# MasterBin-IIAU/Unicorn

Hardware: NVIDIA H100
Metric: frames/sec (higher is better)
Workload: dtype bf16

## Files before the change

unicorn_b200/csrc/mlp_fused.cu:

```cuda
#include <algorithm>
#include "uc_ptx.cuh"
#include "uc_common.h"
#include "../../include/unicorn_b200.h"
#include "uc_epilogue.cuh"

namespace uc {

constexpr int kMlpRows = 128;
constexpr int kMlpHC = 64;
constexpr int kMlpConsumers = 2;
constexpr int kMlpThreads = (1 + kMlpConsumers) * 128;

template <int C>
struct MlpCfg {
  static constexpr int KB = (C + 63) / 64;
  static constexpr int A_BYTES = KB * kMlpRows * 128;
  static constexpr int W1_BYTES = KB * kMlpHC * 128;
  static constexpr int NH = C > 256 ? 2 : 1;
  static constexpr int N2 = C / NH;
  static constexpr int W2_BYTES = N2 * 128;
  static constexpr int NCHUNK = 4 * C / kMlpHC;
  static constexpr int STEPS = NH * NCHUNK;
  static constexpr int AS = C <= 192 ? 2 : 1;
  static constexpr int WS = C <= 256 ? 2 : 1;
  static constexpr int SMEM = AS * A_BYTES + WS * (W1_BYTES + W2_BYTES) + 1024 + 512;
  static constexpr int CPT = C / 16;
};

struct alignas(64) MlpParams {
  CUtensorMap tmA, tmW1, tmW2;
  const float* c1;
  const float* b2;
  const float* gamma;
  uint16_t* x;
  int M, m_tiles;
  float ln_eps;
};

enum { A_FULL = 0, A_EMPTY = 2, W1_FULL = 4, W1_EMPTY = 6, W2_FULL = 8, W2_EMPTY = 10, MLP_NBARS = 12 };

template <int C>
__global__ void __launch_bounds__(kMlpThreads, 1) convnext_mlp_kernel(const __grid_constant__ MlpParams p) {
  using Cfg = MlpCfg<C>;
  extern __shared__ uint8_t smem_raw[];
  uint8_t* smem = reinterpret_cast<uint8_t*>((reinterpret_cast<uintptr_t>(smem_raw) + 1023) & ~uintptr_t(1023));
  uint8_t* sA = smem;
  uint8_t* sW1 = sA + Cfg::AS * Cfg::A_BYTES;
  uint8_t* sW2 = sW1 + Cfg::WS * Cfg::W1_BYTES;
  uint64_t* bar = reinterpret_cast<uint64_t*>(sW2 + Cfg::WS * Cfg::W2_BYTES);
  const int wg = threadIdx.x >> 7, warp = threadIdx.x >> 5, lane = threadIdx.x & 31;

  if (threadIdx.x == 0) {
    prefetch_tmap(&p.tmA);
    prefetch_tmap(&p.tmW1);
    prefetch_tmap(&p.tmW2);
    for (int i = 0; i < 2; ++i) {
      mbar_init(&bar[A_FULL + i], 1);
      mbar_init(&bar[A_EMPTY + i], kMlpConsumers);
      mbar_init(&bar[W1_FULL + i], 1);
      mbar_init(&bar[W1_EMPTY + i], kMlpConsumers);
      mbar_init(&bar[W2_FULL + i], 1);
      mbar_init(&bar[W2_EMPTY + i], kMlpConsumers);
    }
    fence_barrier_init();
  }
  __syncthreads();
  pdl_wait();
  pdl_launch_dependents();

  const int n_local = (p.m_tiles - static_cast<int>(blockIdx.x) + static_cast<int>(gridDim.x) - 1) / static_cast<int>(gridDim.x);
  auto tile_of = [&](int i) { return static_cast<int>(blockIdx.x) + i * static_cast<int>(gridDim.x); };

  if (wg == 0) {
    regs_dealloc<40>();
    if (warp != 0) return;
    auto load_a = [&](int i) {
      const int ab = i % Cfg::AS;
      mbar_wait(&bar[A_EMPTY + ab], ((i / Cfg::AS) & 1) ^ 1);
      if (elect_one()) {
        mbar_arrive_expect_tx(&bar[A_FULL + ab], Cfg::A_BYTES);
#pragma unroll
        for (int kb = 0; kb < Cfg::KB; ++kb)
          tma_load_2d(sA + ab * Cfg::A_BYTES + kb * (kMlpRows * 128), &p.tmA, &bar[A_FULL + ab], kb * 64, tile_of(i) * kMlpRows);
      }
      __syncwarp();
    };
    auto load_w = [&](int g) {
      const int s = g % Cfg::WS, ph = (g / Cfg::WS) & 1, j = g % Cfg::NCHUNK, nh = (g / Cfg::NCHUNK) % Cfg::NH;
      mbar_wait(&bar[W1_EMPTY + s], ph ^ 1);
      if (elect_one()) {
        mbar_arrive_expect_tx(&bar[W1_FULL + s], Cfg::W1_BYTES);
#pragma unroll
        for (int kb = 0; kb < Cfg::KB; ++kb)
          tma_load_2d(sW1 + s * Cfg::W1_BYTES + kb * (kMlpHC * 128), &p.tmW1, &bar[W1_FULL + s], kb * 64, j * kMlpHC);
      }
      __syncwarp();
      mbar_wait(&bar[W2_EMPTY + s], ph ^ 1);
      if (elect_one()) {
        mbar_arrive_expect_tx(&bar[W2_FULL + s], Cfg::W2_BYTES);
        tma_load_2d(sW2 + s * Cfg::W2_BYTES, &p.tmW2, &bar[W2_FULL + s], j * kMlpHC, nh * Cfg::N2);
      }
      __syncwarp();
    };
    const int total = n_local * Cfg::STEPS;
    if (n_local > 0) load_a(0);
    for (int g = 0; g < total; ++g) {
      load_w(g);
      const int i = g / Cfg::STEPS, r = g % Cfg::STEPS;
      if (r == (Cfg::AS == 2 ? 0 : Cfg::STEPS - 1) && i + 1 < n_local) load_a(i + 1);
    }
    return;
  }
  regs_alloc<232>();
  const int c = wg - 1, ct = threadIdx.x & 127;
  const int g8 = lane >> 2, t = lane & 3;
  const int rl = (warp & 3) * 16 + g8;
  const int lr = c * 64 + (ct >> 1), lp = ct & 1;
  auto layer_norm_tile = [&](int ab) {
    uint8_t* a = sA + ab * Cfg::A_BYTES + lr * 128;
    auto chunk_ptr = [&](int cc) {
      const int gc = lp * Cfg::CPT + cc;
      return reinterpret_cast<uint4*>(a + (gc >> 3) * (kMlpRows * 128) + (((gc & 7) ^ (lr & 7)) << 4));
    };
    float s1 = 0.f;
#pragma unroll 4
    for (int cc = 0; cc < Cfg::CPT; ++cc) {
      const uint4 v = *chunk_ptr(cc);
      s1 += (bf16lo(v.x) + bf16hi(v.x)) + (bf16lo(v.y) + bf16hi(v.y)) + (bf16lo(v.z) + bf16hi(v.z)) + (bf16lo(v.w) + bf16hi(v.w));
    }
    s1 += __shfl_xor_sync(0xffffffffu, s1, 1);
    const float mean = s1 * (1.f / C);
    float s2 = 0.f;
#pragma unroll 4
    for (int cc = 0; cc < Cfg::CPT; ++cc) {
      const uint4 v = *chunk_ptr(cc);
      const uint32_t w[4] = {v.x, v.y, v.z, v.w};
#pragma unroll
      for (int e = 0; e < 4; ++e) {
        const float d0 = bf16lo(w[e]) - mean, d1 = bf16hi(w[e]) - mean;
        s2 = fmaf(d0, d0, s2);
        s2 = fmaf(d1, d1, s2);
      }
    }
    s2 += __shfl_xor_sync(0xffffffffu, s2, 1);
    const float rstd = rsqrtf(s2 * (1.f / C) + p.ln_eps);
#pragma unroll 4
    for (int cc = 0; cc < Cfg::CPT; ++cc) {
      uint4* ptr = chunk_ptr(cc);
      const uint4 v = *ptr;
      const uint32_t w[4] = {v.x, v.y, v.z, v.w};
      uint32_t o[4];
#pragma unroll
      for (int e = 0; e < 4; ++e) o[e] = pack2_fast((bf16lo(w[e]) - mean) * rstd, (bf16hi(w[e]) - mean) * rstd, false);
      *ptr = make_uint4(o[0], o[1], o[2], o[3]);
    }
    fence_proxy_async();
    named_sync(1 + c, 128);
  };
  const uint64_t a_desc0 = wgmma_desc_sw128(smem_u32(sA + c * 64 * 128)), w1_desc0 = wgmma_desc_sw128(smem_u32(sW1));
  const uint64_t w2_desc0 = wgmma_desc_sw128(smem_u32(sW2));
  float acc2[Cfg::N2 / 2];
  int g = 0;
  for (int i = 0; i < n_local; ++i) {
    const int ab = i % Cfg::AS;
    mbar_wait(&bar[A_FULL + ab], (i / Cfg::AS) & 1);
    layer_norm_tile(ab);
#pragma unroll 1
   for (int nh = 0; nh < Cfg::NH; ++nh) {
    for (int j = 0; j < Cfg::NCHUNK; ++j, ++g) {
      const int ws = g % Cfg::WS, wph = (g / Cfg::WS) & 1;
      float acc1[kMlpHC / 2];
      mbar_wait(&bar[W1_FULL + ws], wph);
      wgmma_fence();
#pragma unroll
      for (int kb = 0; kb < Cfg::KB; ++kb) {
        const uint64_t ad = a_desc0 + static_cast<uint64_t>((ab * Cfg::A_BYTES + kb * (kMlpRows * 128)) >> 4);
        const uint64_t bd = w1_desc0 + static_cast<uint64_t>((ws * Cfg::W1_BYTES + kb * (kMlpHC * 128)) >> 4);
#pragma unroll
        for (int k = 0; k < 4; ++k) wgmma_ss<kMlpHC, false>(acc1, ad + 2 * k, bd + 2 * k, (kb | k) != 0 ? 1u : 0u);
      }
      wgmma_commit();
      wgmma_wait<0>();
      wgmma_fence_regs(acc1);
      if (ct == 0) {
        mbar_arrive(&bar[W1_EMPTY + ws]);
        if (nh == Cfg::NH - 1 && j == Cfg::NCHUNK - 1) mbar_arrive(&bar[A_EMPTY + ab]);
      }
      uint32_t hf[4][4];
#pragma unroll
      for (int kk = 0; kk < 4; ++kk) {
#pragma unroll
        for (int half = 0; half < 2; ++half) {
          const int i8 = 2 * kk + half;
          const float2 bb = __ldg(reinterpret_cast<const float2*>(p.c1 + j * kMlpHC + 8 * i8 + 2 * t));
          const f32x2 h0 = gelu2(add2(pk2(acc1[4 * i8], acc1[4 * i8 + 1]), pk2(bb.x, bb.y)));
          const f32x2 h1 = gelu2(add2(pk2(acc1[4 * i8 + 2], acc1[4 * i8 + 3]), pk2(bb.x, bb.y)));
          hf[kk][2 * half] = pack2_fast(lo2(h0), hi2(h0), false);
          hf[kk][2 * half + 1] = pack2_fast(lo2(h1), hi2(h1), false);
        }
      }
      mbar_wait(&bar[W2_FULL + ws], wph);
      wgmma_fence();
      const uint64_t bd2 = w2_desc0 + static_cast<uint64_t>((ws * Cfg::W2_BYTES) >> 4);
#pragma unroll
      for (int kk = 0; kk < 4; ++kk) wgmma_rs_bf16<Cfg::N2>(acc2, hf[kk], bd2 + 2 * kk, (j | kk) != 0 ? 1u : 0u);
      wgmma_commit();
      wgmma_wait<0>();
      wgmma_fence_regs(acc2);
      if (ct == 0) mbar_arrive(&bar[W2_EMPTY + ws]);
    }
    const long grow0 = static_cast<long>(tile_of(i)) * kMlpRows + c * 64 + rl;
#pragma unroll
    for (int i8 = 0; i8 < Cfg::N2 / 8; ++i8) {
      const int col = nh * Cfg::N2 + 8 * i8 + 2 * t;
      const float2 b = __ldg(reinterpret_cast<const float2*>(p.b2 + col)), gm = __ldg(reinterpret_cast<const float2*>(p.gamma + col));
#pragma unroll
      for (int h = 0; h < 2; ++h) {
        const long grow = grow0 + 8 * h;
        if (grow < p.M) {
          uint32_t* xp = reinterpret_cast<uint32_t*>(p.x + grow * C + col);
          const uint32_t rw = *xp;
          f32x2 v = add2(pk2(acc2[4 * i8 + 2 * h], acc2[4 * i8 + 2 * h + 1]), pk2(b.x, b.y));
          v = mul2(v, pk2(gm.x, gm.y));
          v = add2(v, pk2(bf16lo(rw), bf16hi(rw)));
          *xp = pack2_fast(lo2(v), hi2(v), false);
        }
      }
    }
   }
  }
}

template <int C>
static int launch_mlp(MlpParams& p, cudaStream_t stream) {
  using Cfg = MlpCfg<C>;
  static PerDeviceFlag attr_dev;
  bool& attr = attr_dev.get();
  auto kern = convnext_mlp_kernel<C>;
  if (!attr) {
    cudaError_t e = cudaFuncSetAttribute(kern, cudaFuncAttributeMaxDynamicSharedMemorySize, Cfg::SMEM);
    if (e != cudaSuccess) return set_error(static_cast<int>(e), "uc_convnext_mlp: cudaFuncSetAttribute: %s", cudaGetErrorString(e));
    attr = true;
  }
  const int grid = std::min(p.m_tiles, num_sms());
  cudaError_t e = launch_pdl(kern, dim3(grid), dim3(kMlpThreads), Cfg::SMEM, stream, p);
  if (e != cudaSuccess) return set_error(static_cast<int>(e), "uc_convnext_mlp<%d> launch: %s", C, cudaGetErrorString(e));
  return check_launch("uc_convnext_mlp");
}

}

using namespace uc;

extern "C" int uc_convnext_mlp_supported(int C) { return C == 96 || C == 192 || C == 256 || C == 384; }

extern "C" int uc_convnext_mlp(const void* t_bf16, const void* w1f_bf16, const float* c1, const void* w2_bf16, const float* b2,
                               const float* gamma, void* x_bf16, int M, int C, float ln_eps, void* stream_v) {
  cudaStream_t stream = static_cast<cudaStream_t>(stream_v);
  if (!t_bf16 || !w1f_bf16 || !c1 || !w2_bf16 || !b2 || !gamma || !x_bf16) return set_error(UC_EINVAL, "uc_convnext_mlp: null pointer");
  if (!uc_convnext_mlp_supported(C)) return set_error(UC_EINVAL, "uc_convnext_mlp: C = %d not supported (96, 192, 256, 384)", C);
  if (M < 1) return set_error(UC_EINVAL, "uc_convnext_mlp: empty map");
  if ((reinterpret_cast<uintptr_t>(t_bf16) | reinterpret_cast<uintptr_t>(w1f_bf16) | reinterpret_cast<uintptr_t>(w2_bf16)) & 15 ||
      (reinterpret_cast<uintptr_t>(x_bf16) | reinterpret_cast<uintptr_t>(c1) | reinterpret_cast<uintptr_t>(b2) | reinterpret_cast<uintptr_t>(gamma)) & 31)
    return set_error(UC_EINVAL, "uc_convnext_mlp: t / weights 16-byte, x / biases 32-byte aligned");
  if (t_bf16 == x_bf16) return set_error(UC_EINVAL, "uc_convnext_mlp: t and x must be different maps");
  int rc = ensure_driver();
  if (rc) return rc;
  MlpParams p;
  memset(&p, 0, sizeof(p));
  const uint64_t es = 2;
  {
    uint64_t dims[2] = {static_cast<uint64_t>(C), static_cast<uint64_t>(M)};
    uint64_t strides[1] = {static_cast<uint64_t>(C) * es};
    uint32_t box[2] = {64, kMlpRows};
    rc = encode_tmap(&p.tmA, CU_TENSOR_MAP_DATA_TYPE_BFLOAT16, 2, t_bf16, dims, strides, box);
    if (rc) return rc;
  }
  {
    uint64_t dims[2] = {static_cast<uint64_t>(C), static_cast<uint64_t>(4 * C)};
    uint64_t strides[1] = {static_cast<uint64_t>(C) * es};
    uint32_t box[2] = {64, kMlpHC};
    rc = encode_tmap(&p.tmW1, CU_TENSOR_MAP_DATA_TYPE_BFLOAT16, 2, w1f_bf16, dims, strides, box);
    if (rc) return rc;
  }
  {
    uint64_t dims[2] = {static_cast<uint64_t>(4 * C), static_cast<uint64_t>(C)};
    uint64_t strides[1] = {static_cast<uint64_t>(4 * C) * es};
    uint32_t box[2] = {kMlpHC, static_cast<uint32_t>(C > 256 ? C / 2 : C)};
    rc = encode_tmap(&p.tmW2, CU_TENSOR_MAP_DATA_TYPE_BFLOAT16, 2, w2_bf16, dims, strides, box);
    if (rc) return rc;
  }
  p.c1 = c1; p.b2 = b2; p.gamma = gamma;
  p.x = static_cast<uint16_t*>(x_bf16);
  p.M = M;
  p.m_tiles = (M + kMlpRows - 1) / kMlpRows;
  p.ln_eps = ln_eps;
  return C == 96 ? launch_mlp<96>(p, stream) : C == 192 ? launch_mlp<192>(p, stream) : C == 256 ? launch_mlp<256>(p, stream) : launch_mlp<384>(p, stream);
}
```

unicorn_b200/csrc/uc_ptx.cuh:

```cuda
#pragma once
#include <cuda_runtime.h>
#include <cuda_bf16.h>
#include <cuda_fp16.h>
#include <cuda.h>
#include <stdint.h>
#include <stdio.h>
#include "uc_wgmma.cuh"

namespace uc {

__device__ __forceinline__ uint32_t smem_u32(const void* p) {
  return static_cast<uint32_t>(__cvta_generic_to_shared(p));
}

__device__ __forceinline__ bool elect_one() {
  uint32_t pred;
  asm volatile(
      "{\n\t.reg .pred p;\n\t"
      "elect.sync _|p, 0xffffffff;\n\t"
      "selp.u32 %0, 1, 0, p;\n\t}"
      : "=r"(pred));
  return pred != 0;
}

__device__ __forceinline__ void mbar_init(uint64_t* bar, uint32_t count) {
  asm volatile("mbarrier.init.shared::cta.b64 [%0], %1;" ::"r"(smem_u32(bar)), "r"(count) : "memory");
}
__device__ __forceinline__ void fence_barrier_init() {
  asm volatile("fence.mbarrier_init.release.cluster;" ::: "memory");
}
__device__ __forceinline__ void fence_proxy_async() {
  asm volatile("fence.proxy.async.shared::cta;" ::: "memory");
}
__device__ __forceinline__ void mbar_arrive_expect_tx(uint64_t* bar, uint32_t bytes) {
  asm volatile("mbarrier.arrive.expect_tx.shared::cta.b64 _, [%0], %1;" ::"r"(smem_u32(bar)), "r"(bytes)
               : "memory");
}
__device__ __forceinline__ void mbar_arrive(uint64_t* bar) {
  asm volatile("mbarrier.arrive.shared::cta.b64 _, [%0];" ::"r"(smem_u32(bar)) : "memory");
}
__device__ __forceinline__ bool mbar_try_wait(uint64_t* bar, uint32_t parity) {
  uint32_t ok;
  asm volatile(
      "{\n\t.reg .pred p;\n\t"
      "mbarrier.try_wait.parity.shared::cta.b64 p, [%1], %2;\n\t"
      "selp.u32 %0, 1, 0, p;\n\t}"
      : "=r"(ok)
      : "r"(smem_u32(bar)), "r"(parity)
      : "memory");
  return ok != 0;
}
__device__ __forceinline__ void mbar_wait(uint64_t* bar, uint32_t parity) {
  if (mbar_try_wait(bar, parity)) return;
  long long t0 = clock64();
  uint32_t spins = 0;
  while (!mbar_try_wait(bar, parity)) {
    if ((++spins & 0x3FF) == 0 && (clock64() - t0) > 4000000000LL) __trap();
  }
}

__device__ __forceinline__ void prefetch_tmap(const CUtensorMap* m) {
  asm volatile("prefetch.tensormap [%0];" ::"l"(reinterpret_cast<uint64_t>(m)) : "memory");
}
__device__ __forceinline__ void tma_load_2d(void* smem, const CUtensorMap* m, uint64_t* bar, int c0, int c1) {
  asm volatile(
      "cp.async.bulk.tensor.2d.shared::cluster.global.mbarrier::complete_tx::bytes [%0], [%1, {%3, %4}], [%2];" ::"r"(
          smem_u32(smem)),
      "l"(reinterpret_cast<uint64_t>(m)), "r"(smem_u32(bar)), "r"(c0), "r"(c1)
      : "memory");
}
__device__ __forceinline__ void tma_load_3d(void* smem, const CUtensorMap* m, uint64_t* bar, int c0, int c1, int c2) {
  asm volatile(
      "cp.async.bulk.tensor.3d.shared::cluster.global.mbarrier::complete_tx::bytes [%0], [%1, {%3, %4, %5}], [%2];" ::
          "r"(smem_u32(smem)),
      "l"(reinterpret_cast<uint64_t>(m)), "r"(smem_u32(bar)), "r"(c0), "r"(c1), "r"(c2)
      : "memory");
}
__device__ __forceinline__ void tma_load_4d(void* smem, const CUtensorMap* m, uint64_t* bar, int c0, int c1, int c2,
                                            int c3) {
  asm volatile(
      "cp.async.bulk.tensor.4d.shared::cluster.global.mbarrier::complete_tx::bytes [%0], [%1, {%3, %4, %5, %6}], "
      "[%2];" ::"r"(smem_u32(smem)),
      "l"(reinterpret_cast<uint64_t>(m)), "r"(smem_u32(bar)), "r"(c0), "r"(c1), "r"(c2), "r"(c3)
      : "memory");
}

__device__ __forceinline__ void tma_load_3d_mc(void* smem, const CUtensorMap* m, uint64_t* bar, int c0, int c1, int c2,
                                               uint16_t cta_mask) {
  asm volatile(
      "cp.async.bulk.tensor.3d.shared::cluster.global.mbarrier::complete_tx::bytes.multicast::cluster [%0], [%1, {%3, %4, "
      "%5}], [%2], %6;" ::"r"(smem_u32(smem)),
      "l"(reinterpret_cast<uint64_t>(m)), "r"(smem_u32(bar)), "r"(c0), "r"(c1), "r"(c2), "h"(cta_mask)
      : "memory");
}
__device__ __forceinline__ uint32_t cluster_ctarank() {
  uint32_t r;
  asm volatile("mov.u32 %0, %%cluster_ctarank;" : "=r"(r));
  return r;
}
__device__ __forceinline__ void cluster_sync_all() {
  asm volatile("barrier.cluster.arrive.release.aligned;\nbarrier.cluster.wait.acquire.aligned;" ::: "memory");
}
__device__ __forceinline__ void mbar_arrive_remote(uint64_t* bar, uint32_t rank) {
  asm volatile(
      "{\n\t.reg .b32 ra;\n\t"
      "mapa.shared::cluster.u32 ra, %0, %1;\n\t"
      "mbarrier.arrive.release.cluster.shared::cluster.b64 _, [ra];\n\t}" ::"r"(smem_u32(bar)),
      "r"(rank)
      : "memory");
}

__device__ __forceinline__ void tma_store_4d(const CUtensorMap* m, const void* smem, int c0, int c1, int c2, int c3) {
  asm volatile("cp.async.bulk.tensor.4d.global.shared::cta.bulk_group [%0, {%2, %3, %4, %5}], [%1];" ::"l"(
                   reinterpret_cast<uint64_t>(m)),
               "r"(smem_u32(smem)), "r"(c0), "r"(c1), "r"(c2), "r"(c3)
               : "memory");
}
__device__ __forceinline__ void tma_store_commit() { asm volatile("cp.async.bulk.commit_group;" ::: "memory"); }
__device__ __forceinline__ void tma_store_wait_read() { asm volatile("cp.async.bulk.wait_group.read 0;" ::: "memory"); }
__device__ __forceinline__ void tma_store_wait_all() { asm volatile("cp.async.bulk.wait_group 0;" ::: "memory"); }

__device__ __forceinline__ void wgmma_fence() { asm volatile("wgmma.fence.sync.aligned;" ::: "memory"); }
__device__ __forceinline__ void wgmma_commit() { asm volatile("wgmma.commit_group.sync.aligned;" ::: "memory"); }
template <int N>
__device__ __forceinline__ void wgmma_wait() { asm volatile("wgmma.wait_group.sync.aligned %0;" ::"n"(N) : "memory"); }
template <int K>
__device__ __forceinline__ void wgmma_fence_regs(float (&d)[K]) {
#pragma unroll
  for (int i = 0; i < K; ++i) asm volatile("" : "+f"(d[i])::"memory");
}
template <int R>
__device__ __forceinline__ void regs_dealloc() { asm volatile("setmaxnreg.dec.sync.aligned.u32 %0;" ::"n"(R)); }
template <int R>
__device__ __forceinline__ void regs_alloc() { asm volatile("setmaxnreg.inc.sync.aligned.u32 %0;" ::"n"(R)); }
__device__ __forceinline__ void named_sync(int id, int count) { asm volatile("bar.sync %0, %1;" ::"r"(id), "r"(count) : "memory"); }
__device__ __forceinline__ void named_arrive(int id, int count) { asm volatile("bar.arrive %0, %1;" ::"r"(id), "r"(count) : "memory"); }

__device__ __forceinline__ uint64_t wgmma_desc_sw128(uint32_t smem_addr) {
  uint64_t d = 0;
  d |= static_cast<uint64_t>((smem_addr & 0x3FFFF) >> 4);
  d |= static_cast<uint64_t>(1) << 16;
  d |= static_cast<uint64_t>(1024 >> 4) << 32;
  d |= static_cast<uint64_t>(1) << 62;
  return d;
}

}
```

Baseline: 177.3.

## Software-pipeline fused ConvNeXt MLP GEMM1/GEMM2 and deepen weight staging

Reworks the fused MLP consumer loop so the first GEMM for the next hidden chunk is issued asynchronously while GELU and the second GEMM of the current chunk run, using double-buffered accumulators. This applies to channel counts up to 192. It also deepens the weight ring buffer for small channel counts, stages the first bias vector in shared memory instead of reading it from global each chunk, and batches the residual loads in the epilogue before computing. The cost is more registers and shared memory and more intricate barrier release ordering, plus a change to the A-tile staging count for C=192.

```diff
diff --git a/unicorn_b200/csrc/mlp_fused.cu b/unicorn_b200/csrc/mlp_fused.cu
--- a/unicorn_b200/csrc/mlp_fused.cu
+++ b/unicorn_b200/csrc/mlp_fused.cu
@@ -10,21 +10,26 @@
 constexpr int kMlpHC = 64;
 constexpr int kMlpConsumers = 2;
 constexpr int kMlpThreads = (1 + kMlpConsumers) * 128;
+constexpr int kMlpMaxWS = 4;
 
 template <int C>
 struct MlpCfg {
+  static constexpr int HC = kMlpHC;
   static constexpr int KB = (C + 63) / 64;
   static constexpr int A_BYTES = KB * kMlpRows * 128;
-  static constexpr int W1_BYTES = KB * kMlpHC * 128;
+  static constexpr int W1_BYTES = KB * HC * 128;
   static constexpr int NH = C > 256 ? 2 : 1;
   static constexpr int N2 = C / NH;
-  static constexpr int W2_BYTES = N2 * 128;
-  static constexpr int NCHUNK = 4 * C / kMlpHC;
+  static constexpr int W2_BYTES = N2 * HC * 2;
+  static constexpr int NCHUNK = 4 * C / HC;
   static constexpr int STEPS = NH * NCHUNK;
-  static constexpr int AS = C <= 192 ? 2 : 1;
-  static constexpr int WS = C <= 256 ? 2 : 1;
-  static constexpr int SMEM = AS * A_BYTES + WS * (W1_BYTES + W2_BYTES) + 1024 + 512;
+  static constexpr int AS = C == 96 ? 2 : 1;
+  static constexpr int WS = C == 96 ? 4 : C == 192 ? 3 : C == 256 ? 2 : 1;
+  static constexpr bool PIPE = C <= 192;
+  static constexpr int SMEM = AS * A_BYTES + WS * (W1_BYTES + W2_BYTES) + 1024 + 512 + 4 * C * 4;
   static constexpr int CPT = C / 16;
+  static_assert((!PIPE || NCHUNK % 2 == 0) && WS <= kMlpMaxWS, "the pipelined chunk loop is unrolled by two");
+  static_assert(SMEM <= 227 * 1024, "shared memory per block");
 };
 
 struct alignas(64) MlpParams {
@@ -37,7 +42,10 @@
   float ln_eps;
 };
 
-enum { A_FULL = 0, A_EMPTY = 2, W1_FULL = 4, W1_EMPTY = 6, W2_FULL = 8, W2_EMPTY = 10, MLP_NBARS = 12 };
+enum {
+  A_FULL = 0, A_EMPTY = 2, W1_FULL = 4, W1_EMPTY = W1_FULL + kMlpMaxWS, W2_FULL = W1_EMPTY + kMlpMaxWS, W2_EMPTY = W2_FULL + kMlpMaxWS,
+  MLP_NBARS = W2_EMPTY + kMlpMaxWS
+};
 
 template <int C>
 __global__ void __launch_bounds__(kMlpThreads, 1) convnext_mlp_kernel(const __grid_constant__ MlpParams p) {
@@ -48,6 +56,7 @@
   uint8_t* sW1 = sA + Cfg::AS * Cfg::A_BYTES;
   uint8_t* sW2 = sW1 + Cfg::WS * Cfg::W1_BYTES;
   uint64_t* bar = reinterpret_cast<uint64_t*>(sW2 + Cfg::WS * Cfg::W2_BYTES);
+  float* sC1 = reinterpret_cast<float*>(bar + 64);
   const int wg = threadIdx.x >> 7, warp = threadIdx.x >> 5, lane = threadIdx.x & 31;
 
   if (threadIdx.x == 0) {
@@ -57,6 +66,8 @@
     for (int i = 0; i < 2; ++i) {
       mbar_init(&bar[A_FULL + i], 1);
       mbar_init(&bar[A_EMPTY + i], kMlpConsumers);
+    }
+    for (int i = 0; i < Cfg::WS; ++i) {
       mbar_init(&bar[W1_FULL + i], 1);
       mbar_init(&bar[W1_EMPTY + i], kMlpConsumers);
       mbar_init(&bar[W2_FULL + i], 1);
@@ -92,13 +103,13 @@
         mbar_arrive_expect_tx(&bar[W1_FULL + s], Cfg::W1_BYTES);
 #pragma unroll
         for (int kb = 0; kb < Cfg::KB; ++kb)
-          tma_load_2d(sW1 + s * Cfg::W1_BYTES + kb * (kMlpHC * 128), &p.tmW1, &bar[W1_FULL + s], kb * 64, j * kMlpHC);
+          tma_load_2d(sW1 + s * Cfg::W1_BYTES + kb * (Cfg::HC * 128), &p.tmW1, &bar[W1_FULL + s], kb * 64, j * Cfg::HC);
       }
       __syncwarp();
       mbar_wait(&bar[W2_EMPTY + s], ph ^ 1);
       if (elect_one()) {
         mbar_arrive_expect_tx(&bar[W2_FULL + s], Cfg::W2_BYTES);
-        tma_load_2d(sW2 + s * Cfg::W2_BYTES, &p.tmW2, &bar[W2_FULL + s], j * kMlpHC, nh * Cfg::N2);
+        tma_load_2d(sW2 + s * Cfg::W2_BYTES, &p.tmW2, &bar[W2_FULL + s], j * Cfg::HC, nh * Cfg::N2);
       }
       __syncwarp();
     };
@@ -113,6 +124,9 @@
   }
   regs_alloc<232>();
   const int c = wg - 1, ct = threadIdx.x & 127;
+  for (int k = threadIdx.x - 128; k < 4 * C; k += kMlpConsumers * 128) sC1[k] = p.c1[k];
+  named_sync(3, kMlpConsumers * 128);
+  const uint32_t c1_s = smem_u32(sC1);
   const int g8 = lane >> 2, t = lane & 3;
   const int rl = (warp & 3) * 16 + g8;
   const int lr = c * 64 + (ct >> 1), lp = ct & 1;
@@ -160,70 +174,128 @@
   const uint64_t a_desc0 = wgmma_desc_sw128(smem_u32(sA + c * 64 * 128)), w1_desc0 = wgmma_desc_sw128(smem_u32(sW1));
   const uint64_t w2_desc0 = wgmma_desc_sw128(smem_u32(sW2));
   float acc2[Cfg::N2 / 2];
+  float acc1[2][Cfg::HC / 2];
+  uint32_t hf[2][Cfg::HC / 16][4];
   int g = 0;
   for (int i = 0; i < n_local; ++i) {
     const int ab = i % Cfg::AS;
     mbar_wait(&bar[A_FULL + ab], (i / Cfg::AS) & 1);
     layer_norm_tile(ab);
+    auto gemm1 = [&](float (&acc)[Cfg::HC / 2], int gs) {
+      const int ws = gs % Cfg::WS;
+      mbar_wait(&bar[W1_FULL + ws], (gs / Cfg::WS) & 1);
+      wgmma_fence();
+#pragma unroll
+      for (int kb = 0; kb < Cfg::KB; ++kb) {
+        const uint64_t ad = a_desc0 + static_cast<uint64_t>((ab * Cfg::A_BYTES + kb * (kMlpRows * 128)) >> 4);
+        const uint64_t bd = w1_desc0 + static_cast<uint64_t>((ws * Cfg::W1_BYTES + kb * (Cfg::HC * 128)) >> 4);
+#pragma unroll
+        for (int k = 0; k < 4; ++k) wgmma_ss<Cfg::HC, false>(acc, ad + 2 * k, bd + 2 * k, (kb | k) != 0 ? 1u : 0u);
+      }
+      wgmma_commit();
+    };
+    auto gelu_chunk = [&](const float (&acc)[Cfg::HC / 2], uint32_t (&h)[Cfg::HC / 16][4], int j) {
+#pragma unroll
+      for (int kk = 0; kk < Cfg::HC / 16; ++kk) {
+#pragma unroll
+        for (int half = 0; half < 2; ++half) {
+          const int i8 = 2 * kk + half;
+          float2 bb;
+          asm volatile("ld.shared.v2.f32 {%0, %1}, [%2];" : "=f"(bb.x), "=f"(bb.y) : "r"(c1_s + 4 * (j * Cfg::HC + 8 * i8 + 2 * t)));
+          const f32x2 h0 = gelu2(add2(pk2(acc[4 * i8], acc[4 * i8 + 1]), pk2(bb.x, bb.y)));
+          const f32x2 h1 = gelu2(add2(pk2(acc[4 * i8 + 2], acc[4 * i8 + 3]), pk2(bb.x, bb.y)));
+          h[kk][2 * half] = pack2_fast(lo2(h0), hi2(h0), false);
+          h[kk][2 * half + 1] = pack2_fast(lo2(h1), hi2(h1), false);
+        }
+      }
+    };
+    auto gemm2 = [&](const uint32_t (&h)[Cfg::HC / 16][4], int gs, int j) {
+      const int ws = gs % Cfg::WS;
+      mbar_wait(&bar[W2_FULL + ws], (gs / Cfg::WS) & 1);
+      wgmma_fence();
+      const uint64_t bd2 = w2_desc0 + static_cast<uint64_t>((ws * Cfg::W2_BYTES) >> 4);
+#pragma unroll
+      for (int kk = 0; kk < Cfg::HC / 16; ++kk) wgmma_rs_bf16<Cfg::N2>(acc2, h[kk], bd2 + 2 * kk, (j | kk) != 0 ? 1u : 0u);
+      wgmma_commit();
+    };
 #pragma unroll 1
    for (int nh = 0; nh < Cfg::NH; ++nh) {
-    for (int j = 0; j < Cfg::NCHUNK; ++j, ++g) {
-      const int ws = g % Cfg::WS, wph = (g / Cfg::WS) & 1;
-      float acc1[kMlpHC / 2];
-      mbar_wait(&bar[W1_FULL + ws], wph);
-      wgmma_fence();
-#pragma unroll
-      for (int kb = 0; kb < Cfg::KB; ++kb) {
-        const uint64_t ad = a_desc0 + static_cast<uint64_t>((ab * Cfg::A_BYTES + kb * (kMlpRows * 128)) >> 4);
-        const uint64_t bd = w1_desc0 + static_cast<uint64_t>((ws * Cfg::W1_BYTES + kb * (kMlpHC * 128)) >> 4);
-#pragma unroll
-        for (int k = 0; k < 4; ++k) wgmma_ss<kMlpHC, false>(acc1, ad + 2 * k, bd + 2 * k, (kb | k) != 0 ? 1u : 0u);
-      }
-      wgmma_commit();
+    const int g0 = g;
+    if constexpr (!Cfg::PIPE) {
+      for (int j = 0; j < Cfg::NCHUNK; ++j) {
+        gemm1(acc1[0], g0 + j);
+        wgmma_wait<0>();
+        wgmma_fence_regs(acc1[0]);
+        if (ct == 0) {
+          mbar_arrive(&bar[W1_EMPTY + (g0 + j) % Cfg::WS]);
+          if (nh == Cfg::NH - 1 && j == Cfg::NCHUNK - 1) mbar_arrive(&bar[A_EMPTY + ab]);
+        }
+        gelu_chunk(acc1[0], hf[0], j);
+        gemm2(hf[0], g0 + j, j);
+        wgmma_wait<0>();
+        wgmma_fence_regs(acc2);
+        if (ct == 0) mbar_arrive(&bar[W2_EMPTY + (g0 + j) % Cfg::WS]);
+      }
+    } else {
+      gemm1(acc1[0], g0);
       wgmma_wait<0>();
-      wgmma_fence_regs(acc1);
-      if (ct == 0) {
-        mbar_arrive(&bar[W1_EMPTY + ws]);
-        if (nh == Cfg::NH - 1 && j == Cfg::NCHUNK - 1) mbar_arrive(&bar[A_EMPTY + ab]);
-      }
-      uint32_t hf[4][4];
-#pragma unroll
-      for (int kk = 0; kk < 4; ++kk) {
-#pragma unroll
-        for (int half = 0; half < 2; ++half) {
-          const int i8 = 2 * kk + half;
-          const float2 bb = __ldg(reinterpret_cast<const float2*>(p.c1 + j * kMlpHC + 8 * i8 + 2 * t));
-          const f32x2 h0 = gelu2(add2(pk2(acc1[4 * i8], acc1[4 * i8 + 1]), pk2(bb.x, bb.y)));
-          const f32x2 h1 = gelu2(add2(pk2(acc1[4 * i8 + 2], acc1[4 * i8 + 3]), pk2(bb.x, bb.y)));
-          hf[kk][2 * half] = pack2_fast(lo2(h0), hi2(h0), false);
-          hf[kk][2 * half + 1] = pack2_fast(lo2(h1), hi2(h1), false);
-        }
-      }
-      mbar_wait(&bar[W2_FULL + ws], wph);
-      wgmma_fence();
-      const uint64_t bd2 = w2_desc0 + static_cast<uint64_t>((ws * Cfg::W2_BYTES) >> 4);
-#pragma unroll
-      for (int kk = 0; kk < 4; ++kk) wgmma_rs_bf16<Cfg::N2>(acc2, hf[kk], bd2 + 2 * kk, (j | kk) != 0 ? 1u : 0u);
-      wgmma_commit();
+      wgmma_fence_regs(acc1[0]);
+      if (ct == 0) mbar_arrive(&bar[W1_EMPTY + g0 % Cfg::WS]);
+#pragma unroll 1
+      for (int jj = 0; jj < Cfg::NCHUNK; jj += 2) {
+#pragma unroll
+        for (int q = 0; q < 2; ++q) {
+          const int j = jj + q;
+          if (j + 1 < Cfg::NCHUNK) gemm1(acc1[q ^ 1], g0 + j + 1);
+          gelu_chunk(acc1[q], hf[q], j);
+          gemm2(hf[q], g0 + j, j);
+          wgmma_wait<1>();
+          wgmma_fence_regs(acc1[q ^ 1]);
+          fence_regs_u32(hf[q ^ 1]);
+          if (ct == 0) {
+            if (j >= 1) mbar_arrive(&bar[W2_EMPTY + (g0 + j - 1) % Cfg::WS]);
+            if (j + 1 < Cfg::NCHUNK) {
+              mbar_arrive(&bar[W1_EMPTY + (g0 + j + 1) % Cfg::WS]);
+              if (nh == Cfg::NH - 1 && j + 2 == Cfg::NCHUNK) mbar_arrive(&bar[A_EMPTY + ab]);
+            }
+          }
+        }
+      }
       wgmma_wait<0>();
       wgmma_fence_regs(acc2);
-      if (ct == 0) mbar_arrive(&bar[W2_EMPTY + ws]);
-    }
+      fence_regs_u32(hf[1]);
+      if (ct == 0) mbar_arrive(&bar[W2_EMPTY + (g0 + Cfg::NCHUNK - 1) % Cfg::WS]);
+    }
+    g += Cfg::NCHUNK;
+    constexpr int EB = 4;
     const long grow0 = static_cast<long>(tile_of(i)) * kMlpRows + c * 64 + rl;
 #pragma unroll
-    for (int i8 = 0; i8 < Cfg::N2 / 8; ++i8) {
-      const int col = nh * Cfg::N2 + 8 * i8 + 2 * t;
-      const float2 b = __ldg(reinterpret_cast<const float2*>(p.b2 + col)), gm = __ldg(reinterpret_cast<const float2*>(p.gamma + col));
-#pragma unroll
-      for (int h = 0; h < 2; ++h) {
-        const long grow = grow0 + 8 * h;
-        if (grow < p.M) {
-          uint32_t* xp = reinterpret_cast<uint32_t*>(p.x + grow * C + col);
-          const uint32_t rw = *xp;
-          f32x2 v = add2(pk2(acc2[4 * i8 + 2 * h], acc2[4 * i8 + 2 * h + 1]), pk2(b.x, b.y));
-          v = mul2(v, pk2(gm.x, gm.y));
-          v = add2(v, pk2(bf16lo(rw), bf16hi(rw)));
-          *xp = pack2_fast(lo2(v), hi2(v), false);
+    for (int i0 = 0; i0 < Cfg::N2 / 8; i0 += EB) {
+      uint32_t rw[EB][2];
+#pragma unroll
+      for (int e = 0; e < EB; ++e) {
+#pragma unroll
+        for (int h = 0; h < 2; ++h) {
+          const long grow = grow0 + 8 * h;
+          if (i0 + e < Cfg::N2 / 8 && grow < p.M)
+            rw[e][h] = *reinterpret_cast<const uint32_t*>(p.x + grow * C + nh * Cfg::N2 + 8 * (i0 + e) + 2 * t);
+        }
+      }
+#pragma unroll
+      for (int e = 0; e < EB; ++e) {
+        const int i8 = i0 + e;
+        if (i8 >= Cfg::N2 / 8) break;
+        const int col = nh * Cfg::N2 + 8 * i8 + 2 * t;
+        const float2 b = __ldg(reinterpret_cast<const float2*>(p.b2 + col)), gm = __ldg(reinterpret_cast<const float2*>(p.gamma + col));
+#pragma unroll
+        for (int h = 0; h < 2; ++h) {
+          const long grow = grow0 + 8 * h;
+          if (grow < p.M) {
+            f32x2 v = add2(pk2(acc2[4 * i8 + 2 * h], acc2[4 * i8 + 2 * h + 1]), pk2(b.x, b.y));
+            v = mul2(v, pk2(gm.x, gm.y));
+            v = add2(v, pk2(bf16lo(rw[e][h]), bf16hi(rw[e][h])));
+            *reinterpret_cast<uint32_t*>(p.x + grow * C + col) = pack2_fast(lo2(v), hi2(v), false);
+          }
         }
       }
     }
diff --git a/unicorn_b200/csrc/uc_ptx.cuh b/unicorn_b200/csrc/uc_ptx.cuh
--- a/unicorn_b200/csrc/uc_ptx.cuh
+++ b/unicorn_b200/csrc/uc_ptx.cuh
@@ -129,6 +129,13 @@
 #pragma unroll
   for (int i = 0; i < K; ++i) asm volatile("" : "+f"(d[i])::"memory");
 }
+template <int K>
+__device__ __forceinline__ void fence_regs_u32(uint32_t (&a)[K][4]) {
+#pragma unroll
+  for (int i = 0; i < K; ++i)
+#pragma unroll
+    for (int e = 0; e < 4; ++e) asm volatile("" : "+r"(a[i][e])::"memory");
+}
 template <int R>
 __device__ __forceinline__ void regs_dealloc() { asm volatile("setmaxnreg.dec.sync.aligned.u32 %0;" ::"n"(R)); }
 template <int R>
```

Result: faster. 180.8, median of 6 (+2.0%).
